# Fannollost/Ray-and-pathtracer

Hardware: AMD Instinct MI355X
Metric: Mrays/s at 1920×1080×64spp (higher is better)
Workload: dtype f32; 1 GPU; config3: pretty_tlas, 1920x1080, 64 spp, path integrator; parallelism=row-interleaved pixel shard x1 + accumulator gather to rank 0, sampler=uniform hemisphere (renderer.cpp:181)

## Files before the change

### profiles/pmc_summary.py

```python
#!/usr/bin/env python3
import csv, glob, os, sys, collections, json
root = sys.argv[1]
tot = collections.defaultdict(lambda: collections.defaultdict(float))
dur = collections.defaultdict(lambda: collections.defaultdict(float))
seen = collections.defaultdict(set)
for f in glob.glob(os.path.join(root, "*", "*", "*counter_collection.csv")):
    pas = f.split(os.sep)[-3]
    for r in csv.DictReader(open(f)):
        k = r["Kernel_Name"]
        if "rtd::" not in k or ("<true" in k and "k_shade_s" not in k):
            continue
        k = k.split("rtd::")[1].split("(")[0]
        tot[k][r["Counter_Name"]] += float(r["Counter_Value"])
        key = (pas, r["Dispatch_Id"])
        if key not in seen[k]:
            seen[k].add(key)
            dur[k][pas] += (int(r["End_Timestamp"]) - int(r["Start_Timestamp"]))
out = {}
for k in sorted(tot):
    n = {p: len([1 for (pp, _) in seen[k] if pp == p]) for p in dur[k]}
    out[k] = {"launches": max(n.values()), "ms_by_pass": {p: round(v / 1e6, 3) for p, v in dur[k].items()}, "counters": dict(tot[k])}
json.dump(out, sys.stdout, indent=1)
```

### ray-and-pathtracer_amd/csrc/rt_api.hip

```cpp
#include "rt_ctx.h"
#include "rt_layout.h"

extern "C" {

int rt_device_count(void)
{
	int n = 0;
	if (hipGetDeviceCount(&n) != hipSuccess) return 0;
	return n;
}

const char* rt_last_error(const rt_ctx* ctx) { return ctx ? ctx->err.c_str() : g_err.c_str(); }

int rt_device_pci_bus_id(int device, char* out, int cap)
{
	if (!out || cap < 16) return fail(nullptr, RT_E_ARG, "rt_device_pci_bus_id: a buffer of at least 16 bytes");
	int n = 0;
	if (hipGetDeviceCount(&n) != hipSuccess || device < 0 || device >= n) return fail(nullptr, RT_E_NODEVICE, "rt_device_pci_bus_id: device %d of %d", device, n);
	if (hipDeviceGetPCIBusId(out, cap, device) != hipSuccess) return fail(nullptr, RT_E_HIP, "hipDeviceGetPCIBusId(%d) failed", device);
	return RT_OK;
}

rt_ctx* rt_create(int device, int width, int height)
{
// ... 2 lines not shown
	if (hipGetDeviceCount(&n) != hipSuccess || n <= 0) { fail(nullptr, RT_E_NODEVICE, "rt_create: no HIP device (this library has no CPU path)"); return nullptr; }
	if (device < 0 || device >= n) { fail(nullptr, RT_E_ARG, "rt_create: device %d of %d", device, n); return nullptr; }
	if (hipSetDevice(device) != hipSuccess) { fail(nullptr, RT_E_HIP, "hipSetDevice(%d) failed", device); return nullptr; }
	hipDeviceProp_t prop;
	if (hipGetDeviceProperties(&prop, device) != hipSuccess) { fail(nullptr, RT_E_HIP, "hipGetDeviceProperties failed"); return nullptr; }
	if (strncmp(prop.gcnArchName, "gfx950", 6) != 0) { fail(nullptr, RT_E_NODEVICE, "rt_create: device %d is %s, this library is built for gfx950 only", device, prop.gcnArchName); return nullptr; }
	rt_ctx* c = new rt_ctx();
	c->device = device, c->width = width, c->height = height;
	read_knobs(c->knobs);
	bool ok = hipStreamCreate(&c->stream) == hipSuccess;
	ok = ok && hipMalloc((void**)&c->accum, (size_t)width * height * sizeof(float4)) == hipSuccess;
	ok = ok && hipMemset(c->accum, 0, (size_t)width * height * sizeof(float4)) == hipSuccess;
	c->gridBlocks = prop.multiProcessorCount * 8;
	{
		const int capBlocks = RT_GRID_CAP;
		auto resident = [&](const void* fn) { int b = 0; if (hipOccupancyMaxActiveBlocksPerMultiprocessor(&b, fn, RT_BLOCK, 0) != hipSuccess || b < 1) b = 1; if (b > 8) b = 8; if (capBlocks >= 1 && b > capBlocks) b = capBlocks; return b * prop.multiProcessorCount; };
		const int e0 = std::min(resident((const void*)k_extend<false, false>), resident((const void*)k_extend<false, true>)), e1 = std::min(resident((const void*)k_extend<true, false>), resident((const void*)k_extend<true, true>));
		const int c0 = resident((const void*)k_connect<false>), c1 = resident((const void*)k_connect<true>);
		c->slot.gridExtend = e0 < e1 ? e0 : e1, c->slot.gridConnect = c0 < c1 ? c0 : c1;
		c->slot.gridConnectWide = resident((const void*)k_connect<false, true>);
		c->slot.gridLeftover = std::min(resident((const void*)k_connect<false, false, true>), prop.multiProcessorCount);
		c->dense.gridExtend = std::min(resident((const void*)k_extend_s<false>), resident((const void*)k_extend_s<true>));
		c->dense.gridConnect = std::min(resident((const void*)k_connect_s<false>), resident((const void*)k_connect_s<true>));
		c->dense.gridConnectWide = resident((const void*)k_connect_s<false, true>);
		c->dense.gridLeftover = std::min(resident((const void*)k_connect_s<false, false, true>), prop.multiProcessorCount);
		c->dense.gridConnectWide8 = resident((const void*)k_connect_s<false, false, false, true>);
		c->dense.gridTraverse = resident((const void*)k_traverse_s);
		c->dense.gridTable = std::min(resident((const void*)k_primary_table<false>), resident((const void*)k_primary_table<true>));
		c->dense.gridBounce = std::min(resident((const void*)k_bounce_table<false>), resident((const void*)k_bounce_table<true>));
		c->mega.grid = resident((const void*)k_whitted_mega);
		c->level.grid = resident((const void*)k_whitted_level);
		c->dense.gridShade = std::min(resident((const void*)k_shade_s<false>), resident((const void*)k_shade_s<true>));
		c->dense.gridShadeBounce = resident((const void*)k_shade_s<false, true>);
		c->dense.gridLight = resident((const void*)k_light_s);
		int q = std::min(c->slot.gridConnect, c->slot.gridExtend);
		const void* qk[9] = { (const void*)k_query_nearest<false>, (const void*)k_query_nearest<true>, (const void*)k_query_occluded<false>, (const void*)k_query_occluded<true>, (const void*)k_primary_hits<false>, (const void*)k_primary_hits<true>,
		                      (const void*)k_query_occluded<false, true>, (const void*)k_query_occluded<false, false, true>, (const void*)k_query_occluded<false, false, false, true> };
		for (int i = 0; i < 9; i++) { const int r = resident(qk[i]); if (r < q) q = r; }
		c->gridQuery = q;
		c->gridAovs = std::min(q, std::min(resident((const void*)k_primary_aovs<false>), resident((const void*)k_primary_aovs<true>)));
	}
	ok = ok && hipMalloc((void**)&c->spill, (size_t)(RT_STACK_MAX - RT_STACK_ROWS_MIN) * c->gridBlocks * RT_BLOCK * sizeof(uint)) == hipSuccess;
	ok = ok && hipMalloc((void**)&c->flags, (16 + RT_HEADS * RT_HEAD_STRIDE) * sizeof(int)) == hipSuccess;
	ok = ok && hipMemset(c->flags, 0, (16 + RT_HEADS * RT_HEAD_STRIDE) * sizeof(int)) == hipSuccess;
	ok = ok && hipMalloc((void**)&c->counters, 2 * sizeof(DCounters)) == hipSuccess;
	ok = ok && hipMemset(c->counters, 0, 2 * sizeof(DCounters)) == hipSuccess;
	ok = ok && hipHostMalloc((void**)&c->hostCounts, 16 * sizeof(int)) == hipSuccess;
	ok = ok && hipMalloc((void**)&c->gammaLut, 256 * sizeof(float)) == hipSuccess;
	if (ok) {
		const int exact = c->knobs.exactGamma;
		ok = hipMemcpyToSymbol(HIP_SYMBOL(g_exactGamma), &exact, sizeof(int), 0, hipMemcpyHostToDevice) == hipSuccess;
	}
	if (ok) hipLaunchKernelGGL(k_gamma_lut, dim3(1), dim3(256), 0, c->stream, c->gammaLut);
	if (!ok) { fail(nullptr, RT_E_HIP, "rt_create: device allocation failed: %s", hipGetErrorString(hipGetLastError())); rt_destroy(c); return nullptr; }
	const float aspect = (float)width / (float)height;
	rt_camera cam;
	memset(&cam, 0, sizeof(cam));
	cam.cam_pos[0] = 0, cam.cam_pos[1] = 1, cam.cam_pos[2] = -2;
	cam.top_left[0] = -aspect, cam.top_left[1] = 2, cam.top_right[0] = aspect, cam.top_right[1] = 2;
	cam.bottom_left[0] = -aspect, cam.view_angle = 0.25f;
	rt_set_camera(c, &cam);
	return c;
}

void rt_destroy(rt_ctx* c)
{
	if (!c) return;
// ... 119 lines not shown
	if (rc != RT_OK) return rc;
	const uint64_t *pa = (const uint64_t*)&a, *pb = (const uint64_t*)&b;
	uint64_t* po = (uint64_t*)out;
	for (int i = 0; i < 8; i++) po[i] = pa[i] + pb[i];
	return RT_OK;
}
int rt_set_profiling(rt_ctx* c, int profiling) { if (!c) return RT_E_ARG; prof_collect(c); c->profiling = profiling != 0; return RT_OK; }
int rt_get_profile(rt_ctx* c, rt_profile* out, int reset)
{
	if (!c || !out) return fail(c, RT_E_ARG, "rt_get_profile: null argument");
	prof_collect(c);
	*out = c->prof;
	if (reset) memset(&c->prof, 0, sizeof(c->prof));
	return RT_OK;
}
#include "rt_api_qlearn.inc"

#ifndef RT_EXTRA_FLAGS
#define RT_EXTRA_FLAGS ""
#endif
#define RT_STR2(x) #x
#define RT_STR(x) RT_STR2(x)
const char* rt_build_info(void)
{
	return "flags=[" RT_EXTRA_FLAGS "] RT_PAIR_REPEAT=" RT_STR(RT_PAIR_REPEAT) " RT_CONNECT_REPEAT=" RT_STR(RT_CONNECT_REPEAT) " RT_HEADS=" RT_STR(RT_HEADS)
	       " RT_HEADS_PROBE=" RT_STR(RT_HEADS_PROBE) " RT_EXTEND_WAVES=" RT_STR(RT_EXTEND_WAVES) " RT_CONNECT_WAVES=" RT_STR(RT_CONNECT_WAVES)
	       " RT_SHADE_S_WAVES=" RT_STR(RT_SHADE_S_WAVES) " RT_STACK_ROWS_MIN=" RT_STR(RT_STACK_ROWS_MIN) " RT_SHORT_QUEUE_RAYS=" RT_STR(RT_SHORT_QUEUE_RAYS)
	       " RT_CHUNK_MIN=" RT_STR(RT_CHUNK_MIN) " RT_LDS_WORDS=" RT_STR(RT_LDS_WORDS);
}
const char* rt_tuning_info(rt_ctx* c)
{
	if (!c) return "";
	char buf[768];
	snprintf(buf, sizeof(buf), "stream=%d decide=%d fuse=%d refill=%d refill_any=%d stepmin=%d stepmin_any=%d stepmin_xform=%d pairagain=%d pairagain_any=%d drain=%d drain_any=%d shade_lds=%d gamma_lut=%d exact_gamma=%d defer_gamma=%d wide=%d wide8=%d mega=%d mega_levels=%d mega_lpt=%d qlearn=%d tlas_lds=%d stack_rows=%d slots=%d primary_table=%d primary_table_min=%d bounce_table=%d",
	         c->knobs.stream, c->knobs.decide, c->knobs.fuse, RT_REFILL, RT_REFILL_ANY, RT_STEPMIN, RT_STEPMIN_ANY, RT_STEPMIN_XFORM,
	         RT_PAIRAGAIN, RT_PAIRAGAIN_ANY, RT_DRAIN_LANES, RT_DRAIN_LANES_ANY, c->knobs.shadeLds, c->S.gammaLut ? 1 : 0, c->knobs.exactGamma, c->knobs.deferGamma, c->S.wide ? 1 : 0, c->S.wide8 ? 1 : 0, c->knobs.mega, c->knobs.megaLevels, c->knobs.megaLpt, c->Qt.on,
	         c->S.tlasLds, c->S.stackRows, slot_budget(c), c->knobs.primaryTable, c->knobs.tableMin, c->knobs.bounceTable);
	c->tuningInfo = buf;
	return c->tuningInfo.c_str();
}

int rt_synchronize(rt_ctx* c)
{
	if (!c) return RT_E_ARG;
	HIPCHK(c, hipSetDevice(c->device));
	HIPCHK(c, hipStreamSynchronize(c->stream));
	return RT_OK;
}

}
```

### ray-and-pathtracer_amd/csrc/rt_api_render.inc

```
static int ensure_state(rt_ctx* c, int nSlots, bool pend)
{
	rt_ctx::SlotState& pl = c->slot;
	const bool wide = c->S.wide != nullptr;
	if (pl.stateSlots >= nSlots && pl.stateLights == c->S.nLights && (pl.statePend || !pend) && (pl.stateWide || !wide)) { pl.P.nSlots = nSlots; return RT_OK; }
	HIPCHK(c, hipStreamSynchronize(c->stream));
	pl.free_state();
	PathState P{};
	const size_t n = (size_t)nSlots;
	for (int b = 0; b < 2; b++) { HIPCHK(c, dalloc(pl.allocs, &P.O[b], n)); HIPCHK(c, dalloc(pl.allocs, &P.D[b], n)); }
	for (int b = 0; b < 2; b++) { HIPCHK(c, dalloc(pl.allocs, &P.hitN[b], n)); HIPCHK(c, dalloc(pl.allocs, &P.hitId[b], n)); }
	HIPCHK(c, dalloc(pl.allocs, &P.hitP, n));
	HIPCHK(c, dalloc(pl.allocs, &P.W, n));
	HIPCHK(c, dalloc(pl.allocs, &P.E, n));
	HIPCHK(c, dalloc(pl.allocs, &P.L, n));
	HIPCHK(c, dalloc(pl.allocs, &P.sh, n * (size_t)(c->S.nLights + 1)));
	HIPCHK(c, dalloc(pl.allocs, &P.vis, n * (size_t)(c->S.nLights + 1)));
	if (pend) {
		HIPCHK(c, dalloc(pl.allocs, &P.pend, n * RT_PEND_CAP * 4));
		HIPCHK(c, dalloc(pl.allocs, &P.pendCount, n));
	}
	Queues Q{};
	HIPCHK(c, dalloc(pl.allocs, &P.status, n + 16));
	HIPCHK(c, dalloc(pl.allocs, &Q.active, n));
	HIPCHK(c, dalloc(pl.allocs, &Q.shadow, n));
// ... 341 lines not shown
	prof_begin(c, K_QUERY, st);
	if (c->counting) hipLaunchKernelGGL(k_primary_table<true>, dim3(grid), dim3(RT_BLOCK), 0, st, c->S, c->C, d.tab, 0.001f, tuning(c), c->spill, c->flags + 16, &d.T.counts[SC_FLAG], c->counters);
	else hipLaunchKernelGGL(k_primary_table<false>, dim3(grid), dim3(RT_BLOCK), 0, st, c->S, c->C, d.tab, 0.001f, tuning(c), c->spill, c->flags + 16, &d.T.counts[SC_FLAG], c->counters);
	if (withBounce) {
		HIPCHK(c, hipMemsetAsync(c->flags + 16, 0, RT_HEADS * RT_HEAD_STRIDE * sizeof(int), st));
		const int gridB = std::min((int)((2 * records + RT_CHUNK - 1) / RT_CHUNK / 4 + 1), d.gridBounce);
		if (c->counting) hipLaunchKernelGGL(k_bounce_table<true>, dim3(gridB), dim3(RT_BLOCK), 0, st, c->S, c->C, d.tab, d.btab, 0.001f, tuning(c), c->spill, c->flags + 16, &d.T.counts[SC_FLAG], c->counters);
		else hipLaunchKernelGGL(k_bounce_table<false>, dim3(gridB), dim3(RT_BLOCK), 0, st, c->S, c->C, d.tab, d.btab, 0.001f, tuning(c), c->spill, c->flags + 16, &d.T.counts[SC_FLAG], c->counters);
		d.bounceGen = c->sceneGen;
	}
	prof_end(c, st);
	d.tableGen = c->sceneGen;
	*use = true, *bounce = withBounce;
	return RT_OK;
}
static int run_rounds_stream(rt_ctx* c, const RenderParams& R, int rounds)
{
	const float t_min = 0.001f;
	const int grid = c->gridBlocks;
	const unsigned mixedMax = c->knobs.mixedMax;
	const bool mixed = !c->counting && (c->knobs.fuse == 1 || (c->knobs.fuse < 0 && R.nSamples < mixedMax)) &&
	                   (unsigned long long)R.nSamples * (unsigned)(c->S.nLights + 1) < 0x7FFFFFFFull;
	const bool twoStreams = !mixed && (c->knobs.fuse < 0 ? R.nSamples < 100000000u : c->knobs.fuse != 0);
	const StreamState& T = c->dense.T;
	hipStream_t st = c->stream, sb = twoStreams ? c->dense.side : c->stream;
	const int cnt = c->counting ? 1 : 0;
	const int n = (int)R.nSamples;
	bool table = false, bounce = false;
	{
		const int rc = primary_table_for(c, R, st, &table, &bounce);
		if (rc != RT_OK) return rc;
	}
	bounce = bounce && c->knobs.bounceTable != 0 && !c->Qt.on;
	prof_begin(c, K_GENERATE, st);
	if (table) hipLaunchKernelGGL(k_generate_t, dim3((n + RT_BLOCK - 1) / RT_BLOCK), dim3(RT_BLOCK), 0, st, c->S, c->C, R, T, c->dense.tab, rounds == 1 ? 1 : 0, cnt);
	else hipLaunchKernelGGL(k_generate_s, dim3((n + RT_BLOCK - 1) / RT_BLOCK), dim3(RT_BLOCK), 0, st, c->S, c->C, R, T, rounds == 1 ? 1 : 0, c->knobs.decide, cnt);
	prof_end(c, st);
	bool pendingJoin = false;
	for (int round = 0; round < rounds; round++) {
		const int last = round + 1 == rounds ? 1 : 0, lastNext = round + 2 == rounds ? 1 : 0;
		if (!(table && round == 0)) {
			hipLaunchKernelGGL(k_compact_s, dim3(grid / 2), dim3(RT_COMPACT_BLOCK), 0, st, T, round);
			tail_probe_reset(st);
			prof_begin(c, K_EXTEND, st);
			if (mixed && round > 0) hipLaunchKernelGGL(k_traverse_s, dim3(c->dense.gridTraverse), dim3(RT_BLOCK), 0, st, c->S, T, round, last, t_min, tuning(c), c->spill);
			else if (c->counting) hipLaunchKernelGGL((k_extend_s<true>), dim3(c->dense.gridExtend), dim3(RT_BLOCK), 0, st, c->S, T, round & 1, last, t_min, tuning(c), c->spill, c->counters);
			else hipLaunchKernelGGL((k_extend_s<false>), dim3(c->dense.gridExtend), dim3(RT_BLOCK), 0, st, c->S, T, round & 1, last, t_min, tuning(c), c->spill, c->counters);
			prof_end(c, st);
			tail_probe_print(st, "extend_s", round);
		}
		if (mixed && round > 0) {
			prof_begin(c, K_SHADE, st);
			hipLaunchKernelGGL(k_light_s, dim3(c->dense.gridLight), dim3(RT_BLOCK), 0, st, c->S, R, T, round - 1, 0, c->knobs.shadeLds);
			prof_end(c, st);
		}
		hipLaunchKernelGGL(k_assign, dim3(grid / 2), dim3(RT_COMPACT_BLOCK), 0, st, T, round);
		if (pendingJoin) { HIPCHK(c, hipStreamWaitEvent(st, c->dense.join, 0)); pendingJoin = false; }
		prof_begin(c, K_SHADE, st);
		if (c->Qt.on) hipLaunchKernelGGL(k_shade_s<true>, dim3(c->dense.gridShade), dim3(RT_BLOCK), 0, st, c->S, c->C, R, T, round, round == 0 ? 1 : 0, last, lastNext, c->knobs.decide, c->knobs.shadeLds, cnt, c->Qt, BounceTable{}, 0);
		else if (bounce && round == 0 && !last) hipLaunchKernelGGL((k_shade_s<false, true>), dim3(c->dense.gridShadeBounce), dim3(RT_BLOCK), 0, st, c->S, c->C, R, T, round, 1, last, lastNext, c->knobs.decide, c->knobs.shadeLds, cnt, c->Qt, c->dense.btab, c->knobs.bounceTable);
		else hipLaunchKernelGGL(k_shade_s<false>, dim3(c->dense.gridShade), dim3(RT_BLOCK), 0, st, c->S, c->C, R, T, round, round == 0 ? 1 : 0, last, lastNext, c->knobs.decide, c->knobs.shadeLds, cnt, c->Qt, BounceTable{}, 0);
		prof_end(c, st);
		if (mixed && !last) continue;
		if (twoStreams) {
			HIPCHK(c, hipEventRecord(c->dense.fork, st));
			HIPCHK(c, hipStreamWaitEvent(sb, c->dense.fork, 0));
		}
		prof_begin(c, K_CONNECT, sb);
		launch_connect_s(c, sb, T, round, twoStreams ? c->dense.sideSpill : c->spill);
		prof_end(c, sb);
		prof_begin(c, K_SHADE, sb);
		hipLaunchKernelGGL(k_light_s, dim3(c->dense.gridLight), dim3(RT_BLOCK), 0, sb, c->S, R, T, round, last, c->knobs.shadeLds);
		prof_end(c, sb);
		if (twoStreams) { HIPCHK(c, hipEventRecord(c->dense.join, sb)); pendingJoin = true; }
	}
	if (pendingJoin) HIPCHK(c, hipStreamWaitEvent(st, c->dense.join, 0));
	if (cnt) hipLaunchKernelGGL(k_fold_decided, dim3(1), dim3(1), 0, st, c->S, T.counts, c->counters);
	HIPCHK(c, hipMemcpyAsync(c->hostCounts, T.counts, 4 * sizeof(int), hipMemcpyDeviceToHost, st));
	c->hostCounts[4] = 0;
	if (c->Qt.on) {
		const int nq = c->Qt.grid * c->Qt.grid * c->Qt.grid * RT_Q_PATCHES;
		hipLaunchKernelGGL(k_q_fold, dim3((nq + 255) / 256), dim3(256), 0, st, c->Qt);
		HIPCHK(c, hipMemcpyAsync(c->hostCounts + 4, c->Qt.ovf, sizeof(int), hipMemcpyDeviceToHost, st));
	}
	HIPCHK(c, hipStreamSynchronize(st));
	const int* hc = c->hostCounts;
	if (hc[4] != 0) {
		(void)hipMemsetAsync(c->Qt.ovf, 0, sizeof(int), st);
		return fail(c, RT_E_OVERFLOW, "Q-learning sampler: more than %u rewards for one (cell, direction) within one batch of frames: render fewer frames per call", RT_Q_ACC_LIMIT);
	}
	if (hc[3] != 0) (void)hipMemsetAsync(T.counts + 3, 0, sizeof(int), st);
	const int rc = decode_status(c, hc[3], FAM_WAVEFRONT);
	if (rc != RT_OK) { c->dense.tableGen = 0, c->dense.bounceGen = 0; return rc; }
	HIPCHK(c, hipGetLastError());
	return RT_OK;
}
static bool stream_eligible(const rt_ctx* c, int mode, size_t samples)
{
	return (c->knobs.stream || c->Qt.on) && mode == RT_MODE_PATH && !c->pathUnsupported && c->counting != RT_COUNT_REFERENCE && samples <= (size_t)slot_budget(c);
}

static int run_general(rt_ctx* c, const RenderParams& R, bool whitted)
{
	if (whitted) hipLaunchKernelGGL(k_trace_general, dim3(c->gridBlocks), dim3(RT_BLOCK), 0, c->stream, c->S, c->C, R, c->spill, c->flags + 1);
	else hipLaunchKernelGGL(k_sample_general, dim3(c->gridBlocks), dim3(RT_BLOCK), 0, c->stream, c->S, c->C, R, c->spill, c->flags + 1);
// ... 267 lines not shown
```

### ray-and-pathtracer_amd/csrc/rt_ctx.h

```cpp
#pragma once
#include "../../include/rt_amd.h"
#include "rt_kernels.h"
#include "rt_stream.h"
#include "rt_mega.h"
#include "rt_build.h"
#include "rt_instances.h"
#include "rt_triangles.h"
#include "rt_layout.h"
#include "rt_denoise.h"
#include "rt_adaptive.h"
#include "rt_budget.h"
#include "rt_dilate.h"
#include "rt_denoise_var.h"
#include "rt_reproject.h"
#include "rt_gather.h"
#include <algorithm>
#include <cstdarg>
#include <cstdio>
#include <cstring>
#include <cstdlib>
#include <functional>
#include <string>
#include <vector>

using namespace rtd;

#ifndef RT_GRID_CAP
#define RT_GRID_CAP 8
#endif
static std::string g_err;

struct Timer {
	hipEvent_t a = nullptr, b = nullptr;
};

struct Knobs {
	long slots = 0;
	long sampleGiB = 4;
	int exactGamma = 0;
	int wide = -1;
	int wide8 = 0;
	int fuse = -1;
	int stream = 1;
	int decide = 1;
	int mega = 1, megaLpt = 1, megaLevels = 2;
	int deferGamma = 1;
	int shadeLds = 1;
	int tlasLds = 1;
	int gammaLut = 1;
	int primaryTable = 1;
	int tableMin = 12;
	int bounceTable = 7;
	int levelCap = 0;
	unsigned mixedMax = 10000000u;
};
static void read_knobs(Knobs& k)
{
	auto num = [](const char* name, long dflt) { const char* e = getenv(name); return e ? atol(e) : dflt; };
	k.slots = num("RT_SLOTS", 0), k.sampleGiB = num("RT_SAMPLE_GIB", 4) > 0 ? num("RT_SAMPLE_GIB", 4) : 4;
	k.exactGamma = num("RT_EXACT_GAMMA", 0) != 0, k.wide = (int)num("RT_WIDE", -1), k.wide8 = num("RT_WIDE8", 0) != 0;
	{ const long f = num("RT_FUSE", -1); k.fuse = f < 0 ? -1 : (f > 2 ? 2 : (int)f); }
	k.stream = num("RT_STREAM", 1) != 0, k.decide = (int)num("RT_DECIDE", 1) & 3, k.mega = num("RT_MEGA", 1) != 0, k.megaLpt = num("RT_MEGA_LPT", 1) != 0;
	k.megaLevels = (int)num("RT_MEGA_LEVELS", 2), k.deferGamma = num("RT_DEFER_GAMMA", 1) != 0, k.shadeLds = num("RT_SHADE_LDS", 1) != 0;
	k.tlasLds = num("RT_TLAS_LDS", 1) != 0, k.gammaLut = num("RT_GAMMA_LUT", 1) != 0, k.levelCap = (int)num("RT_LEVEL_CAP", 0);
	k.mixedMax = (unsigned)num("RT_MIXED_MAX", 10000000);
	k.primaryTable = num("RT_PRIMARY_TABLE", 1) != 0, k.tableMin = (int)std::max(0l, num("RT_PRIMARY_TABLE_MIN", 12));
	{ const char* e = getenv("RT_BOUNCE_TABLE"); k.bounceTable = e ? (int)atol(e) & 7 : 7; }
	if (k.exactGamma) k.deferGamma = 1;
	static bool warned = false;
	const char* retired[] = { "RT_REFILL", "RT_REFILL_ANY", "RT_STEPMIN", "RT_STEPMIN_ANY", "RT_STEPMIN_XFORM", "RT_PAIRAGAIN", "RT_PAIRAGAIN_ANY", "RT_DRAIN_LANES", "RT_DRAIN_LANES_ANY" };
	for (const char* name : retired)
		if (!warned && getenv(name)) { fprintf(stderr, "rt_amd: %s is a compile-time constant (rebuild with make EXTRA=-D%s=N); the environment variable is ignored\n", name, name); warned = true; }
}

template <typename T>
static hipError_t dalloc(std::vector<void*>& pool, T** p, size_t count)
{
	void* q = nullptr;
	hipError_t e = hipMalloc(&q, count * sizeof(T) > 0 ? count * sizeof(T) : 16);
	if (e == hipSuccess) { pool.push_back(q); *p = (T*)q; }
	return e;
}
static void free_pool(std::vector<void*>& pool)
{
	for (void* p : pool) (void)hipFree(p);
	pool.clear();
}

struct rt_ctx {
	int device = 0, width = 0, height = 0;
	Knobs knobs;
	hipStream_t stream = nullptr;
	std::string err, tuningInfo;
	DScene S{};
	bool sceneLoaded = false;
	std::vector<void*> sceneAllocs;
	int sceneRaytracer = -1;
	bool pathUnsupported = false;
	std::string pathUnsupportedWhy;
	float4* primsOrig = nullptr;
// ... 35 lines not shown
	bool cameraSet = false;
	int pixelFilter = RT_FILTER_REFERENCE;
	rt_lens lens{ 0.0f, 1.0f };
	float4* accum = nullptr;
	bool accumOwned = true;
	struct SlotState {
		PathState P{};
		Queues Q{};
		int stateSlots = 0, stateLights = -1;
		bool statePend = false, stateWide = false;
		std::vector<void*> allocs;
		int gridExtend = 0, gridConnect = 0, gridConnectWide = 0, gridLeftover = 0;
		void free_state() { free_pool(allocs); stateSlots = 0; }
	};
	SlotState slot;
	struct DenseState {
		StreamState T{};
		std::vector<void*> allocs;
		int cap = 0, lights = -1;
		bool wide = false;
		hipStream_t side = nullptr;
		uint* sideSpill = nullptr;
		hipEvent_t fork = nullptr, join = nullptr;
		int gridExtend = 0, gridConnect = 0, gridConnectWide = 0, gridLeftover = 0, gridConnectWide8 = 0, gridTraverse = 0;
		int gridShade = 0, gridLight = 0;
		PrimaryTable tab{};
		std::vector<void*> tabAllocs;
		unsigned long long tableGen = 0;
		unsigned long long tablePending = 0, tablePendingGen = 0;
		int gridTable = 0;
		BounceTable btab{};
		unsigned long long bounceGen = 0;
		int gridBounce = 0, gridShadeBounce = 0;
		void free_state() { free_pool(allocs); cap = 0; }
		void destroy()
		{
			free_state();
			free_pool(tabAllocs);
			if (side) { (void)hipStreamSynchronize(side); (void)hipStreamDestroy(side); }
			if (sideSpill) (void)hipFree(sideSpill);
			if (fork) (void)hipEventDestroy(fork);
			if (join) (void)hipEventDestroy(join);
		}
	};
	DenseState dense;
	struct MegaForm {
		MegaState M{};
		std::vector<void*> allocs;
		int lanes = 0, grid = 0;
		struct Auto { unsigned nSamples = 0; int depth = 0; int tried[2] = { 0, 0 }; float ms[2] = { 0, 0 }; int choice = -1; } pick;
		hipEvent_t ev[2] = { nullptr, nullptr };
		std::vector<void*> orderAllocs;
		uint* cost = nullptr; uint* order = nullptr; uint* hist = nullptr;
		size_t costCap = 0;
		unsigned costSamples = 0, costFirst = 0;
		void free_lanes() { free_pool(allocs); lanes = 0; }
		void free_order() { free_pool(orderAllocs); costCap = 0, costSamples = 0; }
		void destroy()
		{
			free_lanes(), free_order();
			for (int k = 0; k < 2; k++) if (ev[k]) (void)hipEventDestroy(ev[k]);
		}
	};
	MegaForm mega;
	struct LevelForm {
		LevelState V{};
// ... 248 lines not shown
```

### ray-and-pathtracer_amd/csrc/rt_stream.h

```cpp
#pragma once
#include "rt_kernels.h"
#include "rt_qlearn.h"

namespace rtd {

#define CL_TRACE 1
#define CL_LIVE 2
#define CL_CONT 4
#define CL_SHADOW 8

#define SC_N 0
#define SC_FLAG 3
#define SC_SHADOW 4
#define SC_TRACE 7
#define SC_LEFTOVER 8
#define SC_DECIDED 9

struct StreamState {
	float4* O[2];
	float4* D[2];
	float4* hitN[2];
	int2* hitId[2];
	float4* W[2];
	float4* E[2];
// ... 276 lines not shown
}

__global__ void __launch_bounds__(RT_BLOCK) k_generate_t(DScene S, DCamera C, RenderParams R, StreamState T, PrimaryTable P, int last, int counting)
{
	const int e = blockIdx.x * blockDim.x + threadIdx.x;
	const bool valid = e < (int)R.nSamples;
	prepare_round(T, 0, (int)R.nSamples);
	if (valid) {
		const uint sid = R.sampleFirst + (uint)e;
		int px, py;
		uint seed;
		sample_primary_pixel(C, R, sid, px, py, seed);
		RT_CHECK(px >= -1 && px <= C.width && py >= -1 && py <= C.height, 25, &T.counts[SC_FLAG]);
		const size_t i = (size_t)(px + 1) + (size_t)(py + 1) * (size_t)P.w;
		const int4 b = P.B[i];
		const float4 a = P.A[i];
		unsigned char cls = 0;
		if (b.z & PT_FINISHED) {
			if ((b.z & PT_TEXEL) && S.gammaLut) R.samples[sid] = make_float4(S.gammaLut[b.w & 255], S.gammaLut[(b.w >> 8) & 255], S.gammaLut[(b.w >> 16) & 255], 0.0f);
			else store_sample(R, sid, xyz(a));
		} else {
			f3 O, D;
			primary_ray(C, px, py, O, D);
			T.O[0][e] = mk4(O, a.w);
			T.D[0][e] = mk4(D, 0.0f);
			T.hitN[0][e] = a;
			T.hitId[0][e] = make_int2(b.x, b.y);
			cls = (unsigned char)(CL_LIVE | ((last ? b.z >> 4 : b.z) & 15));
		}
		T.cls[0][e] = cls;
	}
	if (counting) flush_decided(T.counts, valid ? 1u : 0u);
}

struct StreamExtendPolicy {
	const DScene& S;
	const StreamState& T;
	int parity, last;
	int* flag;
	__device__ __forceinline__ bool load(int work, f3& O, f3& D, float& tmax, HitRef& head) const
	{
		const int e = (int)ld_stream(T.traceQ + work);
		RT_CHECK(e >= 0 && e < T.cap, 20, flag);
		const float4 o4 = ld_stream(T.O[parity] + e), d4 = ld_stream(T.D[parity] + e);
		O = xyz(o4), D = xyz(d4), tmax = o4.w;
		unpack_head(__float_as_uint(d4.w), head);
		return true;
	}
	__device__ __forceinline__ int slot_of(int work) const { return (int)T.traceQ[work]; }
	__device__ __forceinline__ void store(int work, const HitRef& hit, const f3& , const f3& ) const
	{
		const int e = (int)ld_stream(T.traceQ + work);
		int objIdx, mat, matType;
		f3 normal;
		const StreamState& Tc = T;
		const int par = parity;
		resolve_hit_lazy(S, hit, [&](f3& o, f3& d) { o = xyz(ld_stream(Tc.O[par] + e)), d = xyz(ld_stream(Tc.D[par] + e)); }, objIdx, mat, normal, &matType);
		st_stream(T.hitN[parity] + e, mk4(normal, hit.t));
		st_stream(T.hitId[parity] + e, make_int2(objIdx, mat));
		T.cls[parity][e] = (unsigned char)(CL_LIVE | CL_TRACE | hit_class(S, objIdx, mat, last, matType));
	}
};
template <bool COUNT>
__global__ void __launch_bounds__(RT_BLOCK, RT_EXTEND_WAVES) k_extend_s(DScene S, StreamState T, int parity, int last, float t_min, int tuning, uint* spill, DCounters* counters)
{
	__shared__ __attribute__((aligned(16))) uint ldsStack[RT_LDS_WORDS];
// ... 54 lines not shown
		int inC = cC, inS = cS;
		for (int o = 1; o < 64; o <<= 1) {
			const int tc = __shfl_up(inC, o), ts = __shfl_up(inS, o);
			if ((int)lane >= o) inC += tc, inS += ts;
		}
		const int pc = bc + inC - cC, ps = bs + inS - cS;
		if (e0 < last && (lane & 3) == 0) T.pos[e0 >> 6] = make_int2(pc, ps);
		bc += __shfl(inC, 63), bs += __shfl(inS, 63);
	}
}

#define RT_LDS_MATS 48
#define RT_LDS_BRUTE 24
struct ShadeTables { uint mats[RT_LDS_MATS * 16]; float4 brute[RT_LDS_BRUTE * 4]; uint lights[RT_MAX_LIGHTS * (sizeof(DLight) / 4)]; };
__device__ __forceinline__ void load_tables(DScene& S, ShadeTables& L, int enable)
{
	const bool m = enable && S.nMats <= RT_LDS_MATS, b = enable && S.useTLAS && S.nBruteSph + S.nBrutePla <= RT_LDS_BRUTE && S.nBruteSph + S.nBrutePla > 0;
	const bool l = enable && S.nLights > 0 && S.nLights <= RT_MAX_LIGHTS;
	if (m) for (int i = (int)threadIdx.x; i < S.nMats * 16; i += (int)blockDim.x) L.mats[i] = ((const uint*)S.mats)[i];
	if (b) for (int i = (int)threadIdx.x; i < (S.nBruteSph + S.nBrutePla) * 4; i += (int)blockDim.x) L.brute[i] = S.brute[i];
	if (l) for (int i = (int)threadIdx.x; i < S.nLights * (int)(sizeof(DLight) / 4); i += (int)blockDim.x) L.lights[i] = ((const uint*)S.lights)[i];
	if (m || b || l) __syncthreads();
	if (m) S.mats = (const DMaterial*)L.mats;
	if (b) S.brute = L.brute;
	if (l) S.lights = (const DLight*)L.lights;
}

#ifndef RT_SHADE_S_WAVES
#define RT_SHADE_S_WAVES 5
#endif
#ifndef RT_SHADE_Q_WAVES
#define RT_SHADE_Q_WAVES 5
#endif
template <bool QL, bool BOUNCE = false>
__global__ void __launch_bounds__(RT_BLOCK, QL ? RT_SHADE_Q_WAVES : RT_SHADE_S_WAVES) k_shade_s(DScene S0, DCamera C, RenderParams R, StreamState T, int round, int fresh, int last, int lastNext, int decide, int ldsTables, int counting, QTable Qt, BounceTable Bt, int bounceMask)
{
	__shared__ ShadeTables tables;
	uint nDecided = 0;
	uint qOld = 0;
	const int parity = round & 1;
	prepare_round(T, round + 1, -1);
	DScene S = S0;
	load_tables(S, tables, ldsTables);
	const int pout = 1 - parity;
	const int n = T.counts[SC_N + round % 3];
	const size_t cap = (size_t)T.cap;
	const int nIter = (n + (int)(gridDim.x * blockDim.x) - 1) / (int)(gridDim.x * blockDim.x);
	for (int it = 0; it < nIter; it++) {
		const int e = it * (int)(gridDim.x * blockDim.x) + (int)(blockIdx.x * blockDim.x + threadIdx.x);
		const bool spec = !fresh && e < n;
		float4 o4, d4, hn, e4, w4, l4;
		int2 id;
		const int2 grp = e < n ? T.pos[e >> 6] : make_int2(0, 0);
		if (spec) {
			o4 = T.O[parity][e], d4 = T.D[parity][e], hn = T.hitN[parity][e], id = T.hitId[parity][e];
			e4 = T.E[parity][e], w4 = T.W[parity][e], l4 = T.L[parity][e];
		}
		const unsigned char c = e < n ? T.cls[parity][e] : 0;
		int2 p;
		{
			const unsigned long long mC = __ballot((c & CL_CONT) != 0), mS = __ballot((c & CL_SHADOW) != 0);
			p.x = grp.x + (int)__builtin_amdgcn_mbcnt_hi((uint)(mC >> 32), __builtin_amdgcn_mbcnt_lo((uint)mC, 0u));
			p.y = grp.y + (int)__builtin_amdgcn_mbcnt_hi((uint)(mS >> 32), __builtin_amdgcn_mbcnt_lo((uint)mS, 0u));
		}
		if (c & CL_LIVE) {
			int primaryRec = -1;
			if (!spec) {
				o4 = T.O[parity][e], d4 = T.D[parity][e], hn = T.hitN[parity][e], id = T.hitId[parity][e];
				if constexpr (BOUNCE) {
					int px, py;
					uint s0;
					sample_primary_pixel(C, R, R.sampleFirst + (uint)e, px, py, s0);
					e4 = make_float4(1, 1, 1, __uint_as_float(s0));
					primaryRec = (px + 1) + (py + 1) * Bt.w;
				} else e4 = fresh_energy(C, R, R.sampleFirst + (uint)e);
				w4 = make_float4(1, 1, 1, 0);
				l4 = make_float4(0, 0, 0, __uint_as_float(R.sampleFirst + (uint)e));
			}
			RT_CHECK(!(c & CL_CONT) || (p.x >= 0 && p.x < T.cap && p.y >= 0 && p.y < T.cap), 21, &T.counts[SC_FLAG]);
			const f3 O = xyz(o4), D = xyz(d4), normal = xyz(hn);
			const float t = hn.w;
			f3 W = xyz(w4), E = xyz(e4), Lsum = xyz(l4);
			uint seed = __float_as_uint(e4.w), shadowSeed = 0;
			const f3 I = O + t * D;
			const bool childTraces = !last;
			bool segmentEnds = true, wantShadow = false;
			f3 nO(0.0f), nD(0.0f), nW(0.0f);
			uint nextKey = 0;
			bool deadSample = false;
			int bounceRec = -1;
			const uint keyWord = QL ? (fresh ? (((__float_as_uint(e4.w) & Qt.learnMask) == 0) ? RT_Q_LEARNER : 0u) : __float_as_uint(w4.w)) : 0u;
			const bool learner = (keyWord & RT_Q_LEARNER) != 0;
			const uint prevKey = learner ? (keyWord & ~RT_Q_LEARNER) : 0u;

			f3 term;
			if (terminal_radiance(S, id.x, I, normal, D, term)) {
				Lsum = Lsum + W * term;
				if (QL && prevKey) qOld |= q_reward(Qt, prevKey, q_lum(term));
			} else {
				const DMaterial m = S.mats[id.y];
// ... 23 lines not shown
					wantShadow = S.nLights > 0;
					shadowSeed = seed;
					for (int i = 0; i < S.nLights; i++) {
						const f3 pickedPos = light_position(S.lights[i], false, seed);
						T.shP[(size_t)i * cap + (size_t)p.y] = mk4(pickedPos, 0.0f);
					}
					const f3 albedo(m.albedo[0], m.albedo[1], m.albedo[2]);
					if constexpr (QL) {
						float P;
						int patch;
						const int cell = q_cell(Qt, I);
						const f3 dirQ = q_sample(Qt, cell, seed, P, patch);
						const float c = dot(dirQ, normal);
						nO = I, nD = dirQ;
						if (c > 0) {
							const f3 cos_i(c);
							nW = W * (((1.0f / (16.0f * P)) * (col * cos_i)) * albedo);
							nextKey = learner ? 1u + (uint)cell * RT_Q_PATCHES + (uint)patch : 0u;
						} else {
							deadSample = true;
							if (learner) qOld |= q_reward(Qt, 1u + (uint)cell * RT_Q_PATCHES + (uint)patch, 0.0f);
						}
					} else {
						nO = I;
						hemisphere_bounce(seed, normal, col, albedo, W, nD, nW);
					}
					if (childTraces) segmentEnds = false;
					else Lsum = Lsum + untraced_child(nW);
				}
			}
			RT_CHECK(((c & CL_SHADOW) != 0) == wantShadow && ((c & CL_CONT) != 0) == (!segmentEnds || wantShadow), 22, &T.counts[SC_FLAG]);
			if (wantShadow) {
				T.shI[p.y] = mk4(I, __uint_as_float(shadowSeed));
				T.shX[p.y] = make_int2(e, p.x);
			}
			if (!segmentEnds || wantShadow) {
				T.E[pout][p.x] = mk4(E, __uint_as_float(seed));
				T.L[pout][p.x] = mk4(Lsum, l4.w);
				if (!segmentEnds && deadSample) {
					T.O[pout][p.x] = mk4(nO, 1e34f), T.D[pout][p.x] = mk4(nD, 0.0f);
					T.hitN[pout][p.x] = make_float4(0, 0, 0, 1e34f), T.hitId[pout][p.x] = make_int2(-1, -1);
					T.W[pout][p.x] = make_float4(0, 0, 0, 0);
					T.cls[pout][p.x] = CL_LIVE;
				} else if (!segmentEnds) {
					int4 bb = make_int4(0, 0, 0, 0);
					if constexpr (BOUNCE) {
						RT_CHECK(fresh && primaryRec >= 0 && primaryRec < Bt.n && bounceRec < 2 * Bt.n, 27, &T.counts[SC_FLAG]);
						if (primaryRec >= 0 && primaryRec < Bt.n && bounceRec >= 0) bb = Bt.B[bounceRec];
					}
					if (BOUNCE && (bb.z & BT_PRESENT)) {
						const float4 ba = Bt.A[bounceRec];
						T.hitN[pout][p.x] = ba;
						T.hitId[pout][p.x] = make_int2(bb.x, bb.y);
						T.O[pout][p.x] = mk4(nO, ba.w), T.D[pout][p.x] = mk4(nD, 0.0f);
						T.W[pout][p.x] = mk4(nW, __uint_as_float(nextKey | (keyWord & RT_Q_LEARNER)));
						T.cls[pout][p.x] = (unsigned char)(CL_LIVE | ((lastNext ? bb.z >> 4 : bb.z) & 15));
						nDecided++;
					} else {
						const NewRay nr = emit_ray_s(S, T, pout, p.x, nO, nD, mode_t_min(1), lastNext, false, decide != 0);
						T.W[pout][p.x] = mk4(nW, __uint_as_float(nextKey | (keyWord & RT_Q_LEARNER)));
						T.cls[pout][p.x] = nr.cls;
						nDecided += nr.decided ? 1u : 0u;
					}
				}
			} else store_sample(R, __float_as_uint(l4.w), Lsum);
		}
	}
// ... 33 lines not shown
	int* heads = T.heads + RT_HEADS * RT_HEAD_STRIDE;
	if constexpr (LISTED) {
		ListedPolicy<StreamConnectPolicy> lp{ pol, T.leftover };
		trace_persistent<true, COUNT, false, ListedPolicy<StreamConnectPolicy>>(S, lp, T.counts[SC_LEFTOVER], heads, 0.0f, tuning, ldsStack, spill, &T.counts[SC_FLAG], lc, rays);
	} else
		trace_persistent<true, COUNT, false, StreamConnectPolicy, false, WIDE8 ? 8 : (WIDE ? 4 : 2)>(S, pol, nShadow * S.nLights, heads, 0.0f, tuning, ldsStack, spill, &T.counts[SC_FLAG], lc, rays);
	if (COUNT) flush_counters(counters, lc, 0, rays);
}

struct StreamTraversePolicy {
	StreamExtendPolicy ext;
	StreamConnectPolicy con;
	int nTrace;
	__device__ __forceinline__ bool any_of(int work) const { return work >= nTrace; }
	__device__ __forceinline__ bool load(int work, f3& O, f3& D, float& tmax, HitRef& head) const
	{
		if (work < nTrace) return ext.load(work, O, D, tmax, head);
		return con.load(work - nTrace, O, D, tmax, head);
	}
	__device__ __forceinline__ void store(int work, const HitRef& hit, const f3& O, const f3& D) const { ext.store(work, hit, O, D); }
	__device__ __forceinline__ void store(int work, bool occluded) const { con.store(work - nTrace, occluded); }
};
__global__ void __launch_bounds__(RT_BLOCK, RT_TRAVERSE_WAVES) k_traverse_s(DScene S, StreamState T, int round, int last, float t_min, int tuning, uint* spill)
{
	__shared__ __attribute__((aligned(16))) uint ldsStack[RT_LDS_WORDS];
	LaneCounters lc;
	lc.clear();
	uint rays = 0;
	const int nTrace = T.counts[SC_TRACE], nShadow = T.counts[SC_SHADOW + (round + 2) % 3];
	StreamTraversePolicy pol{ { S, T, round & 1, last, &T.counts[SC_FLAG] }, { T, nShadow > 0 ? nShadow : 1, &T.counts[SC_FLAG] }, nTrace };
	trace_persistent<false, false, false, StreamTraversePolicy, true>(S, pol, nTrace + nShadow * S.nLights, T.heads, t_min, tuning, ldsStack, spill, &T.counts[SC_FLAG], lc, rays);
}

__global__ void RT_LIGHT_BOUNDS k_light_s(DScene S0, RenderParams R, StreamState T, int round, int last, int ldsTables)
{
	__shared__ ShadeTables tables;
	DScene S = S0;
	load_tables(S, tables, ldsTables);
	const int p = round & 1, pout = 1 - p;
	const int n = T.counts[SC_SHADOW + round % 3];
	const size_t cap = (size_t)T.cap;
	for (int s = blockIdx.x * blockDim.x + threadIdx.x; s < n; s += gridDim.x * blockDim.x) {
		const float4 i4 = T.shI[s];
		const int2 x = T.shX[s];
		const int e = x.x, cp = x.y;
		RT_CHECK(e >= 0 && e < T.cap && cp >= 0 && cp < T.cap, 24, &T.counts[SC_FLAG]);
		const float4 n4 = T.hitN[p][e], d4 = T.D[p][e];
		const int mat = T.hitId[p][e].y;
		const f3 W = round == 0 ? f3(1.0f) : xyz(T.W[p][e]);
		const float4 e4 = T.E[pout][cp], l4 = T.L[pout][cp];
		const f3 I = xyz(i4), normal = xyz(n4), D = xyz(d4);
		f3 E = xyz(e4), Lsum = xyz(l4);
		uint seed = __float_as_uint(i4.w);
		const DMaterial m = S.mats[mat];
		const f3 col(m.col[0], m.col[1], m.col[2]);
		f3 direct(0.0f);
		for (int i = 0; i < S.nLights; i++) {
			const f3 pickedPos = light_position(S.lights[i], false, seed);
			const f3 lightRayDirection = normalize(pickedPos - I);
			if (T.vis[(size_t)i * cap + (size_t)s] != 0) continue;
			const f3 att = diffuse_scatter(m, D, lightRayDirection, light_intensity(S.lights[i], I, normal, pickedPos), normal, E);
			direct = direct + direct_term(m, col, att, E);
		}
		const f3 albedo(m.albedo[0], m.albedo[1], m.albedo[2]);
		Lsum = Lsum + W * path_direct(direct, albedo);
		if (last) store_sample(R, __float_as_uint(l4.w), Lsum);
		else {
			if (E.x != e4.x || E.y != e4.y || E.z != e4.z) T.E[pout][cp] = mk4(E, e4.w);
			if (Lsum.x != l4.x || Lsum.y != l4.y || Lsum.z != l4.z) T.L[pout][cp] = mk4(Lsum, l4.w);
		}
	}
}

}
```

Before: 3979 Mrays/s.

## Read round-0 hit data straight from primary table instead of per-sample stream buffers

Adds a round-0 path in which generation writes only the class byte per sample, and the shade and light kernels rebuild origin, direction, hit normal and id from the primary-hit table and camera. This removes the per-sample writes and reads of O/D/hitN/hitId for the first bounce. In exchange, the camera ray is recomputed in the shade and light kernels and shadow records point at table entries. An env knob can disable the path or poison the skipped buffers with memsets for checking.

New measurement: 4031 Mrays/s (median of 6 runs). +1.3%, better.

```diff
diff --git a/profiles/pmc_summary.py b/profiles/pmc_summary.py
--- a/profiles/pmc_summary.py
+++ b/profiles/pmc_summary.py
@@ -8,7 +8,7 @@
     pas = f.split(os.sep)[-3]
     for r in csv.DictReader(open(f)):
         k = r["Kernel_Name"]
-        if "rtd::" not in k or ("<true" in k and "k_shade_s" not in k):
+        if "rtd::" not in k or ("<true" in k and "k_shade_s" not in k and "k_light_s" not in k):
             continue
         k = k.split("rtd::")[1].split("(")[0]
         tot[k][r["Counter_Name"]] += float(r["Counter_Value"])
diff --git a/ray-and-pathtracer_amd/csrc/rt_api.hip b/ray-and-pathtracer_amd/csrc/rt_api.hip
--- a/ray-and-pathtracer_amd/csrc/rt_api.hip
+++ b/ray-and-pathtracer_amd/csrc/rt_api.hip
@@ -58,7 +58,10 @@
 		c->level.grid = resident((const void*)k_whitted_level);
 		c->dense.gridShade = std::min(resident((const void*)k_shade_s<false>), resident((const void*)k_shade_s<true>));
 		c->dense.gridShadeBounce = resident((const void*)k_shade_s<false, true>);
-		c->dense.gridLight = resident((const void*)k_light_s);
+		c->dense.gridShadeDirect = resident((const void*)k_shade_s<false, false, true>);
+		c->dense.gridShadeDirectBounce = resident((const void*)k_shade_s<false, true, true>);
+		c->dense.gridLight = resident((const void*)k_light_s<false>);
+		c->dense.gridLightDirect = resident((const void*)k_light_s<true>);
 		int q = std::min(c->slot.gridConnect, c->slot.gridExtend);
 		const void* qk[9] = { (const void*)k_query_nearest<false>, (const void*)k_query_nearest<true>, (const void*)k_query_occluded<false>, (const void*)k_query_occluded<true>, (const void*)k_primary_hits<false>, (const void*)k_primary_hits<true>,
 		                      (const void*)k_query_occluded<false, true>, (const void*)k_query_occluded<false, false, true>, (const void*)k_query_occluded<false, false, false, true> };
@@ -244,10 +247,10 @@
 {
 	if (!c) return "";
 	char buf[768];
-	snprintf(buf, sizeof(buf), "stream=%d decide=%d fuse=%d refill=%d refill_any=%d stepmin=%d stepmin_any=%d stepmin_xform=%d pairagain=%d pairagain_any=%d drain=%d drain_any=%d shade_lds=%d gamma_lut=%d exact_gamma=%d defer_gamma=%d wide=%d wide8=%d mega=%d mega_levels=%d mega_lpt=%d qlearn=%d tlas_lds=%d stack_rows=%d slots=%d primary_table=%d primary_table_min=%d bounce_table=%d",
+	snprintf(buf, sizeof(buf), "stream=%d decide=%d fuse=%d refill=%d refill_any=%d stepmin=%d stepmin_any=%d stepmin_xform=%d pairagain=%d pairagain_any=%d drain=%d drain_any=%d shade_lds=%d gamma_lut=%d exact_gamma=%d defer_gamma=%d wide=%d wide8=%d mega=%d mega_levels=%d mega_lpt=%d qlearn=%d tlas_lds=%d stack_rows=%d slots=%d primary_table=%d primary_table_min=%d bounce_table=%d round0_entries=%d",
 	         c->knobs.stream, c->knobs.decide, c->knobs.fuse, RT_REFILL, RT_REFILL_ANY, RT_STEPMIN, RT_STEPMIN_ANY, RT_STEPMIN_XFORM,
 	         RT_PAIRAGAIN, RT_PAIRAGAIN_ANY, RT_DRAIN_LANES, RT_DRAIN_LANES_ANY, c->knobs.shadeLds, c->S.gammaLut ? 1 : 0, c->knobs.exactGamma, c->knobs.deferGamma, c->S.wide ? 1 : 0, c->S.wide8 ? 1 : 0, c->knobs.mega, c->knobs.megaLevels, c->knobs.megaLpt, c->Qt.on,
-	         c->S.tlasLds, c->S.stackRows, slot_budget(c), c->knobs.primaryTable, c->knobs.tableMin, c->knobs.bounceTable);
+	         c->S.tlasLds, c->S.stackRows, slot_budget(c), c->knobs.primaryTable, c->knobs.tableMin, c->knobs.bounceTable, c->knobs.round0Entries);
 	c->tuningInfo = buf;
 	return c->tuningInfo.c_str();
 }
diff --git a/ray-and-pathtracer_amd/csrc/rt_api_render.inc b/ray-and-pathtracer_amd/csrc/rt_api_render.inc
--- a/ray-and-pathtracer_amd/csrc/rt_api_render.inc
+++ b/ray-and-pathtracer_amd/csrc/rt_api_render.inc
@@ -397,10 +397,18 @@
 		if (rc != RT_OK) return rc;
 	}
 	bounce = bounce && c->knobs.bounceTable != 0 && !c->Qt.on;
+	const bool direct = table && !c->Qt.on && !c->C.fisheye && c->knobs.round0Entries != 1;
 	prof_begin(c, K_GENERATE, st);
-	if (table) hipLaunchKernelGGL(k_generate_t, dim3((n + RT_BLOCK - 1) / RT_BLOCK), dim3(RT_BLOCK), 0, st, c->S, c->C, R, T, c->dense.tab, rounds == 1 ? 1 : 0, cnt);
+	if (direct) hipLaunchKernelGGL(k_generate_c, dim3((n + RT_BLOCK - 1) / RT_BLOCK), dim3(RT_BLOCK), 0, st, c->S, c->C, R, T, c->dense.tab, rounds == 1 ? 1 : 0, cnt);
+	else if (table) hipLaunchKernelGGL(k_generate_t, dim3((n + RT_BLOCK - 1) / RT_BLOCK), dim3(RT_BLOCK), 0, st, c->S, c->C, R, T, c->dense.tab, rounds == 1 ? 1 : 0, cnt);
 	else hipLaunchKernelGGL(k_generate_s, dim3((n + RT_BLOCK - 1) / RT_BLOCK), dim3(RT_BLOCK), 0, st, c->S, c->C, R, T, rounds == 1 ? 1 : 0, c->knobs.decide, cnt);
 	prof_end(c, st);
+	if (direct && c->knobs.round0Entries == 2) {
+		HIPCHK(c, hipMemsetAsync(T.O[0], 0xFF, (size_t)n * sizeof(float4), st));
+		HIPCHK(c, hipMemsetAsync(T.D[0], 0xFF, (size_t)n * sizeof(float4), st));
+		HIPCHK(c, hipMemsetAsync(T.hitN[0], 0xFF, (size_t)n * sizeof(float4), st));
+		HIPCHK(c, hipMemsetAsync(T.hitId[0], 0xFF, (size_t)n * sizeof(int2), st));
+	}
 	bool pendingJoin = false;
 	for (int round = 0; round < rounds; round++) {
 		const int last = round + 1 == rounds ? 1 : 0, lastNext = round + 2 == rounds ? 1 : 0;
@@ -416,15 +424,18 @@
 		}
 		if (mixed && round > 0) {
 			prof_begin(c, K_SHADE, st);
-			hipLaunchKernelGGL(k_light_s, dim3(c->dense.gridLight), dim3(RT_BLOCK), 0, st, c->S, R, T, round - 1, 0, c->knobs.shadeLds);
+			if (direct && round == 1) hipLaunchKernelGGL(k_light_s<true>, dim3(c->dense.gridLightDirect), dim3(RT_BLOCK), 0, st, c->S, R, T, round - 1, 0, c->knobs.shadeLds, c->C, c->dense.tab);
+			else hipLaunchKernelGGL(k_light_s<false>, dim3(c->dense.gridLight), dim3(RT_BLOCK), 0, st, c->S, R, T, round - 1, 0, c->knobs.shadeLds, c->C, PrimaryTable{});
 			prof_end(c, st);
 		}
 		hipLaunchKernelGGL(k_assign, dim3(grid / 2), dim3(RT_COMPACT_BLOCK), 0, st, T, round);
 		if (pendingJoin) { HIPCHK(c, hipStreamWaitEvent(st, c->dense.join, 0)); pendingJoin = false; }
 		prof_begin(c, K_SHADE, st);
-		if (c->Qt.on) hipLaunchKernelGGL(k_shade_s<true>, dim3(c->dense.gridShade), dim3(RT_BLOCK), 0, st, c->S, c->C, R, T, round, round == 0 ? 1 : 0, last, lastNext, c->knobs.decide, c->knobs.shadeLds, cnt, c->Qt, BounceTable{}, 0);
-		else if (bounce && round == 0 && !last) hipLaunchKernelGGL((k_shade_s<false, true>), dim3(c->dense.gridShadeBounce), dim3(RT_BLOCK), 0, st, c->S, c->C, R, T, round, 1, last, lastNext, c->knobs.decide, c->knobs.shadeLds, cnt, c->Qt, c->dense.btab, c->knobs.bounceTable);
-		else hipLaunchKernelGGL(k_shade_s<false>, dim3(c->dense.gridShade), dim3(RT_BLOCK), 0, st, c->S, c->C, R, T, round, round == 0 ? 1 : 0, last, lastNext, c->knobs.decide, c->knobs.shadeLds, cnt, c->Qt, BounceTable{}, 0);
+		if (c->Qt.on) hipLaunchKernelGGL(k_shade_s<true>, dim3(c->dense.gridShade), dim3(RT_BLOCK), 0, st, c->S, c->C, R, T, round, round == 0 ? 1 : 0, last, lastNext, c->knobs.decide, c->knobs.shadeLds, cnt, c->Qt, BounceTable{}, 0, PrimaryTable{});
+		else if (direct && round == 0 && bounce && !last) hipLaunchKernelGGL((k_shade_s<false, true, true>), dim3(c->dense.gridShadeDirectBounce), dim3(RT_BLOCK), 0, st, c->S, c->C, R, T, round, 1, last, lastNext, c->knobs.decide, c->knobs.shadeLds, cnt, c->Qt, c->dense.btab, c->knobs.bounceTable, c->dense.tab);
+		else if (direct && round == 0) hipLaunchKernelGGL((k_shade_s<false, false, true>), dim3(c->dense.gridShadeDirect), dim3(RT_BLOCK), 0, st, c->S, c->C, R, T, round, 1, last, lastNext, c->knobs.decide, c->knobs.shadeLds, cnt, c->Qt, BounceTable{}, 0, c->dense.tab);
+		else if (bounce && round == 0 && !last) hipLaunchKernelGGL((k_shade_s<false, true>), dim3(c->dense.gridShadeBounce), dim3(RT_BLOCK), 0, st, c->S, c->C, R, T, round, 1, last, lastNext, c->knobs.decide, c->knobs.shadeLds, cnt, c->Qt, c->dense.btab, c->knobs.bounceTable, PrimaryTable{});
+		else hipLaunchKernelGGL(k_shade_s<false>, dim3(c->dense.gridShade), dim3(RT_BLOCK), 0, st, c->S, c->C, R, T, round, round == 0 ? 1 : 0, last, lastNext, c->knobs.decide, c->knobs.shadeLds, cnt, c->Qt, BounceTable{}, 0, PrimaryTable{});
 		prof_end(c, st);
 		if (mixed && !last) continue;
 		if (twoStreams) {
@@ -435,7 +446,8 @@
 		launch_connect_s(c, sb, T, round, twoStreams ? c->dense.sideSpill : c->spill);
 		prof_end(c, sb);
 		prof_begin(c, K_SHADE, sb);
-		hipLaunchKernelGGL(k_light_s, dim3(c->dense.gridLight), dim3(RT_BLOCK), 0, sb, c->S, R, T, round, last, c->knobs.shadeLds);
+		if (direct && round == 0) hipLaunchKernelGGL(k_light_s<true>, dim3(c->dense.gridLightDirect), dim3(RT_BLOCK), 0, sb, c->S, R, T, round, last, c->knobs.shadeLds, c->C, c->dense.tab);
+		else hipLaunchKernelGGL(k_light_s<false>, dim3(c->dense.gridLight), dim3(RT_BLOCK), 0, sb, c->S, R, T, round, last, c->knobs.shadeLds, c->C, PrimaryTable{});
 		prof_end(c, sb);
 		if (twoStreams) { HIPCHK(c, hipEventRecord(c->dense.join, sb)); pendingJoin = true; }
 	}
diff --git a/ray-and-pathtracer_amd/csrc/rt_ctx.h b/ray-and-pathtracer_amd/csrc/rt_ctx.h
--- a/ray-and-pathtracer_amd/csrc/rt_ctx.h
+++ b/ray-and-pathtracer_amd/csrc/rt_ctx.h
@@ -51,6 +51,7 @@
 	int primaryTable = 1;
 	int tableMin = 12;
 	int bounceTable = 7;
+	int round0Entries = 0;
 	int levelCap = 0;
 	unsigned mixedMax = 10000000u;
 };
@@ -66,6 +67,7 @@
 	k.mixedMax = (unsigned)num("RT_MIXED_MAX", 10000000);
 	k.primaryTable = num("RT_PRIMARY_TABLE", 1) != 0, k.tableMin = (int)std::max(0l, num("RT_PRIMARY_TABLE_MIN", 12));
 	{ const char* e = getenv("RT_BOUNCE_TABLE"); k.bounceTable = e ? (int)atol(e) & 7 : 7; }
+	{ const char* e = getenv("RT_ROUND0_ENTRIES"); const long v = e ? atol(e) : 0; k.round0Entries = v == 1 || v == 2 ? (int)v : 0; }
 	if (k.exactGamma) k.deferGamma = 1;
 	static bool warned = false;
 	const char* retired[] = { "RT_REFILL", "RT_REFILL_ANY", "RT_STEPMIN", "RT_STEPMIN_ANY", "RT_STEPMIN_XFORM", "RT_PAIRAGAIN", "RT_PAIRAGAIN_ANY", "RT_DRAIN_LANES", "RT_DRAIN_LANES_ANY" };
@@ -167,6 +169,7 @@
 		BounceTable btab{};
 		unsigned long long bounceGen = 0;
 		int gridBounce = 0, gridShadeBounce = 0;
+		int gridShadeDirect = 0, gridShadeDirectBounce = 0, gridLightDirect = 0;
 		void free_state() { free_pool(allocs); cap = 0; }
 		void destroy()
 		{
diff --git a/ray-and-pathtracer_amd/csrc/rt_stream.h b/ray-and-pathtracer_amd/csrc/rt_stream.h
--- a/ray-and-pathtracer_amd/csrc/rt_stream.h
+++ b/ray-and-pathtracer_amd/csrc/rt_stream.h
@@ -332,6 +332,28 @@
 	}
 	if (counting) flush_decided(T.counts, valid ? 1u : 0u);
 }
+__global__ void __launch_bounds__(RT_BLOCK) k_generate_c(DScene S, DCamera C, RenderParams R, StreamState T, PrimaryTable P, int last, int counting)
+{
+	const int e = blockIdx.x * blockDim.x + threadIdx.x;
+	const bool valid = e < (int)R.nSamples;
+	prepare_round(T, 0, (int)R.nSamples);
+	if (valid) {
+		const uint sid = R.sampleFirst + (uint)e;
+		int px, py;
+		uint seed;
+		sample_primary_pixel(C, R, sid, px, py, seed);
+		RT_CHECK(px >= -1 && px <= C.width && py >= -1 && py <= C.height, 25, &T.counts[SC_FLAG]);
+		const size_t i = (size_t)(px + 1) + (size_t)(py + 1) * (size_t)P.w;
+		const int4 b = P.B[i];
+		unsigned char cls = 0;
+		if (b.z & PT_FINISHED) {
+			if ((b.z & PT_TEXEL) && S.gammaLut) R.samples[sid] = make_float4(S.gammaLut[b.w & 255], S.gammaLut[(b.w >> 8) & 255], S.gammaLut[(b.w >> 16) & 255], 0.0f);
+			else store_sample(R, sid, xyz(P.A[i]));
+		} else cls = (unsigned char)(CL_LIVE | ((last ? b.z >> 4 : b.z) & 15));
+		T.cls[0][e] = cls;
+	}
+	if (counting) flush_decided(T.counts, valid ? 1u : 0u);
+}
 
 struct StreamExtendPolicy {
 	const DScene& S;
@@ -452,9 +474,10 @@
 #ifndef RT_SHADE_Q_WAVES
 #define RT_SHADE_Q_WAVES 5
 #endif
-template <bool QL, bool BOUNCE = false>
-__global__ void __launch_bounds__(RT_BLOCK, QL ? RT_SHADE_Q_WAVES : RT_SHADE_S_WAVES) k_shade_s(DScene S0, DCamera C, RenderParams R, StreamState T, int round, int fresh, int last, int lastNext, int decide, int ldsTables, int counting, QTable Qt, BounceTable Bt, int bounceMask)
-{
+template <bool QL, bool BOUNCE = false, bool TABLE0 = false>
+__global__ void __launch_bounds__(RT_BLOCK, QL ? RT_SHADE_Q_WAVES : RT_SHADE_S_WAVES) k_shade_s(DScene S0, DCamera C, RenderParams R, StreamState T, int round, int fresh, int last, int lastNext, int decide, int ldsTables, int counting, QTable Qt, BounceTable Bt, int bounceMask, PrimaryTable P)
+{
+	static_assert(!(QL && TABLE0), "the sampler's round 0 keeps its entries");
 	__shared__ ShadeTables tables;
 	uint nDecided = 0;
 	uint qOld = 0;
@@ -468,7 +491,7 @@
 	const int nIter = (n + (int)(gridDim.x * blockDim.x) - 1) / (int)(gridDim.x * blockDim.x);
 	for (int it = 0; it < nIter; it++) {
 		const int e = it * (int)(gridDim.x * blockDim.x) + (int)(blockIdx.x * blockDim.x + threadIdx.x);
-		const bool spec = !fresh && e < n;
+		const bool spec = !TABLE0 && !fresh && e < n;
 		float4 o4, d4, hn, e4, w4, l4;
 		int2 id;
 		const int2 grp = e < n ? T.pos[e >> 6] : make_int2(0, 0);
@@ -485,7 +508,21 @@
 		}
 		if (c & CL_LIVE) {
 			int primaryRec = -1;
-			if (!spec) {
+			if constexpr (TABLE0) {
+				int px, py;
+				uint s0;
+				sample_primary_pixel(C, R, R.sampleFirst + (uint)e, px, py, s0);
+				primaryRec = (px + 1) + (py + 1) * P.w;
+				RT_CHECK(fresh && round == 0 && primaryRec >= 0 && primaryRec < P.w * P.h && (!BOUNCE || (Bt.w == P.w && Bt.n == P.w * P.h)), 28, &T.counts[SC_FLAG]);
+				hn = P.A[primaryRec];
+				id = *(const int2*)(P.B + primaryRec);
+				f3 o, d;
+				primary_ray_f(C, (float)px, (float)py, o, d);
+				o4 = mk4(o, 0.0f), d4 = mk4(d, 0.0f);
+				e4 = make_float4(1, 1, 1, __uint_as_float(s0));
+				w4 = make_float4(1, 1, 1, 0);
+				l4 = make_float4(0, 0, 0, __uint_as_float(R.sampleFirst + (uint)e));
+			} else if (!spec) {
 				o4 = T.O[parity][e], d4 = T.D[parity][e], hn = T.hitN[parity][e], id = T.hitId[parity][e];
 				if constexpr (BOUNCE) {
 					int px, py;
@@ -575,7 +612,7 @@
 			RT_CHECK(((c & CL_SHADOW) != 0) == wantShadow && ((c & CL_CONT) != 0) == (!segmentEnds || wantShadow), 22, &T.counts[SC_FLAG]);
 			if (wantShadow) {
 				T.shI[p.y] = mk4(I, __uint_as_float(shadowSeed));
-				T.shX[p.y] = make_int2(e, p.x);
+				T.shX[p.y] = make_int2(TABLE0 ? primaryRec : e, p.x);
 			}
 			if (!segmentEnds || wantShadow) {
 				T.E[pout][p.x] = mk4(E, __uint_as_float(seed));
@@ -675,7 +712,8 @@
 	trace_persistent<false, false, false, StreamTraversePolicy, true>(S, pol, nTrace + nShadow * S.nLights, T.heads, t_min, tuning, ldsStack, spill, &T.counts[SC_FLAG], lc, rays);
 }
 
-__global__ void RT_LIGHT_BOUNDS k_light_s(DScene S0, RenderParams R, StreamState T, int round, int last, int ldsTables)
+template <bool TABLE0>
+__global__ void RT_LIGHT_BOUNDS k_light_s(DScene S0, RenderParams R, StreamState T, int round, int last, int ldsTables, DCamera C, PrimaryTable P)
 {
 	__shared__ ShadeTables tables;
 	DScene S = S0;
@@ -687,10 +725,17 @@
 		const float4 i4 = T.shI[s];
 		const int2 x = T.shX[s];
 		const int e = x.x, cp = x.y;
-		RT_CHECK(e >= 0 && e < T.cap && cp >= 0 && cp < T.cap, 24, &T.counts[SC_FLAG]);
-		const float4 n4 = T.hitN[p][e], d4 = T.D[p][e];
-		const int mat = T.hitId[p][e].y;
-		const f3 W = round == 0 ? f3(1.0f) : xyz(T.W[p][e]);
+		RT_CHECK(e >= 0 && e < (TABLE0 ? P.w * P.h : T.cap) && cp >= 0 && cp < T.cap && (!TABLE0 || round == 0), 24, &T.counts[SC_FLAG]);
+		float4 n4, d4;
+		int mat;
+		if constexpr (TABLE0) {
+			n4 = P.A[e];
+			mat = P.B[e].y;
+			f3 o, d;
+			primary_ray_f(C, (float)(e % P.w - 1), (float)(e / P.w - 1), o, d);
+			d4 = mk4(d, 0.0f);
+		} else n4 = T.hitN[p][e], d4 = T.D[p][e], mat = T.hitId[p][e].y;
+		const f3 W = TABLE0 || round == 0 ? f3(1.0f) : xyz(T.W[p][e]);
 		const float4 e4 = T.E[pout][cp], l4 = T.L[pout][cp];
 		const f3 I = xyz(i4), normal = xyz(n4), D = xyz(d4);
 		f3 E = xyz(e4), Lsum = xyz(l4);
```
